# wbhart/mpir-fft

Measured on AMD Instinct MI355X. Metric: limbs/s for new_mpn_mul N×N-bit at 1/2/4/8 MI355X; % HBM roofline, higher is better.
Workload: dtype u64; 1 GPU; C3: new_mpn_mul depth=15 w=4 n1=n2=20312500 limbs (l=2048 limbs/coeff, NC x NR = 256 x 256, trunc=39936); parallelism=single

## Files before the change

include/mpfft.h:

```cpp
#ifndef MPFFT_H
#define MPFFT_H

#include <stddef.h>
#include <stdint.h>

#if !defined(__GMP_H__) && !defined(__MPIR_H__) && !defined(MPFFT_HAVE_MP_TYPES)
typedef uint64_t mp_limb_t;
typedef long mp_size_t;
typedef unsigned long mp_bitcnt_t;
#endif

#define MPFFT_VERSION 2

#define MPFFT_OK 0
#define MPFFT_EINVAL 1
#define MPFFT_ETOOBIG 2
#define MPFFT_EUNSUPPORTED 3
#define MPFFT_ENOMEM 4
#define MPFFT_EHIP 5
#define MPFFT_ENODEV 6

#ifdef __cplusplus
extern "C" {
#endif
// ... 83 lines not shown
    int src, dst;
    int op;
    int field;
    int src_layout, dst_layout;
    long src_off, dst_off, count;
} mpfft_copy;
#define MPFFT_XCHG_COL_TO_ROW 1
#define MPFFT_XCHG_ROW_TO_COL 2
#define MPFFT_LAYOUT_HALO 2
long mpfft_shard_exchange_plan(long n1, long n2, unsigned long depth, unsigned long w, int world, int which,
                               mpfft_copy *out, long cap);
long mpfft_shard_halo_plan(long n1, long n2, unsigned long depth, unsigned long w, int world,
                           mpfft_copy *out, long cap);

int mpfft_mul_multi(uint64_t *r1, const uint64_t *i1, long n1, const uint64_t *i2, long n2,
                    unsigned long depth, unsigned long w, int ngpus, const int *devices);

long mpfft_shard_src_limbs(long n1, long n2, unsigned long depth, unsigned long w, int world);
int mpfft_shard_pack(long n1, long n2, unsigned long depth, unsigned long w, int world, int rank,
                     const uint64_t *a, long na, uint64_t *out);

int mpfft_mul_multi_device(long n1, long n2, unsigned long depth, unsigned long w, int ngpus, const int *devices,
                           const uint64_t *const *d_src1, const uint64_t *const *d_src2, uint64_t *const *d_r,
                           void *const *streams);
int mpfft_multi_release(void);
long mpfft_multi_schedule(long n1, long n2, unsigned long depth, unsigned long w, int world, int calls, char *buf,
                          size_t len);

int mpfft_set_devices(int ngpus, const int *devices, long min_l);
int mpfft_last_ngpus(void);

int mpfft_profile_begin(int max_calls);
int mpfft_stage_kernels(long n1, long n2, unsigned long depth, unsigned long w, char *buf, size_t len);
int mpfft_profile_end(float *stage_ms, int *calls);

const char *mpfft_strerror(int code);
int mpfft_version(void);

void mpfft_fill_random(uint64_t *buf, long cnt, uint64_t seed);

#ifdef __cplusplus
}
#endif

#endif
```

mpir-fft_amd/__init__.py:

```python
import ctypes
import os

import numpy as np

_HERE = os.path.dirname(os.path.abspath(__file__))
_LIBSEL = os.environ.get("MPFFT_LIB", "")
LIB_PATH = os.path.join(_HERE, "libmpfft_diag.so" if _LIBSEL == "diag" else
                        _LIBSEL if _LIBSEL.endswith(".so") else "libmpfft.so")
_lib = None

STAGE_FWD_COLUMNS, STAGE_FWD_ROWS, STAGE_POINTWISE, STAGE_INV_ROWS, STAGE_INV_COLUMNS, \
    STAGE_SCALE, STAGE_COMBINE, STAGE_FOLD_COMBINE = range(8)

_u64p = ctypes.POINTER(ctypes.c_uint64)
_vp = ctypes.c_void_p
_L = ctypes.c_long
_UL = ctypes.c_ulong


class _Shard(ctypes.Structure):
    _fields_ = [("n1", ctypes.c_long), ("n2", ctypes.c_long), ("depth", ctypes.c_ulong), ("w", ctypes.c_ulong),
                ("c0", ctypes.c_int), ("ccount", ctypes.c_int), ("r0", ctypes.c_int), ("rcount", ctypes.c_int),
                ("ccb", ctypes.c_int),
                ("col_dig", ctypes.c_void_p * 2), ("col_cb", ctypes.c_void_p * 2), ("col_top", ctypes.c_void_p * 2),
# ... 250 lines not shown
def alloc_workspace(n1, n2, depth, w, device="cuda"):
    import torch
    nb = workspace_bytes(n1, n2, depth, w)
    if nb == 0:
        raise MpfftError(check_params(n1, n2, depth, w), "workspace")
    return torch.empty(nb, dtype=torch.uint8, device=device)


def mul_device(d_r, d_i1, n1, d_i2, n2, depth, w, ws, stream=None):
    rc = lib().mpfft_mul_device(_ptr(d_r), _ptr(d_i1), n1, _ptr(d_i2), n2, depth, w, _ptr(ws),
                                ws.numel() * ws.element_size(), _stream(stream))
    if rc:
        raise MpfftError(rc, "mpfft_mul_device")


def stage(which, d_i1, d_i2, d_r, n1, n2, depth, w, ws, stream=None):
    rc = lib().mpfft_stage(which, _ptr(d_i1), _ptr(d_i2), _ptr(d_r), n1, n2, depth, w, _ptr(ws),
                           ws.numel() * ws.element_size(), _stream(stream))
    if rc:
        raise MpfftError(rc, f"mpfft_stage({which})")


STAGE_NAMES = ("fwd_columns", "fwd_rows", "pointwise", "inv_rows", "inv_columns", "scale", "combine")


def stage_kernels(n1, n2, depth, w):
    buf = ctypes.create_string_buffer(512)
    rc = lib().mpfft_stage_kernels(n1, n2, depth, w, buf, len(buf))
    if rc:
        raise MpfftError(rc, "mpfft_stage_kernels")
    return dict(zip(STAGE_NAMES, buf.value.decode().split(";")))


def profile_begin(max_calls):
    rc = lib().mpfft_profile_begin(max_calls)
    if rc:
        raise MpfftError(rc, "mpfft_profile_begin")


def profile_end():
    ms = (ctypes.c_float * len(STAGE_NAMES))()
    calls = ctypes.c_int(0)
    rc = lib().mpfft_profile_end(ms, ctypes.byref(calls))
    if rc:
        raise MpfftError(rc, "mpfft_profile_end")
    return dict(zip(STAGE_NAMES, [float(x) for x in ms])), calls.value


def workspace_layout(n1, n2, depth, w):
    out = (ctypes.c_size_t * 8)()
    rc = lib().mpfft_workspace_layout(n1, n2, depth, w, out)
    if rc:
        raise MpfftError(rc, "workspace_layout")
    keys = ("digA", "topA", "cbA", "digB", "topB", "cbB", "slots", "cbw")
    return dict(zip(keys, list(out)))


def workspace_views(ws, n1, n2, depth, w):
    import torch
    P = plan_info(n1, n2, depth, w)
    lay = workspace_layout(n1, n2, depth, w)
    slots, l = lay["slots"], P["l"]
    u8 = ws.view(torch.uint8)

    def dig(off):
        return u8[off:off + slots * l * 8].view(torch.int64).view(slots, l)
# ... 158 lines not shown
```

mpir-fft_amd/csrc/kernels.hpp:

```cpp
#pragma once
#include "coeff.hpp"

struct PassArgs {
    u64 *dig[2];
    u64 *cb[2];
    int *top[2];
    const u64 *src[2];
    long nsrc[2];
    long src_chunk;
    u64 bits1;
    u64 N;
    int l;
    int lbM, lvl0;
    u64 rho;
    long sub_stride, pos_stride;
    int nsub, pos_off;
    int pbb;
    long pbs;
    int sub_off;
    long jNC;
    int zero_from;
    int need;
    int need_lo;
    int tw_mode;
    u64 tw_w;
    int tw_lbR;
    int canon;
    int ngroups;
    int nbuf;
    u64 scale_e;
    int ablate;
    unsigned *zp;
    long zn;
    unsigned long long *dbg;
    int pcarry;
    int pkeep;
    int fill_lo, fill_off;
    u64 fill_rho;
    int grp0;
};

__device__ inline void pass_clear_flags(const PassArgs &a)
{
    if (!a.zp) return;
    const long nt = (long)blockDim.x * blockDim.y * blockDim.z;
    const long nthr = (long)gridDim.x * gridDim.y * gridDim.z * nt;
    const long bid = ((long)blockIdx.z * gridDim.y + blockIdx.y) * gridDim.x + blockIdx.x;
    const long t = bid * nt + ((long)threadIdx.z * blockDim.y + threadIdx.y) * blockDim.x + threadIdx.x;
    for (long i = t; i < a.zn; i += nthr) a.zp[i] = 0u;
}

struct Lds {
    i64 *stage;
    int *edge;
    u64 *scr;
};

__host__ __device__ inline size_t lds_bytes(int l, int rb, int G, int U, int nw)
{
    size_t st = (size_t)rb * 2 * l * sizeof(i64);
    size_t ed = ((size_t)norm_edge_ints(G, U, nw) * sizeof(int) + 15) / 16 * 16;
    return st + ed + (size_t)norm_scr_u64(G, U, nw) * sizeof(u64);
}

template <int U, int G>
__device__ __forceinline__ Lds lds_carve(unsigned char *smem, int l, int rb, int nw)
{
    Lds d;
    d.stage = (i64 *)smem;
    unsigned char *p = smem + (size_t)rb * 2 * l * sizeof(i64);
    d.edge = (int *)p;
// ... 999 lines not shown
```

mpir-fft_amd/csrc/mpfft.hip:

```cpp
#include <hip/hip_runtime.h>
#include <stdint.h>
#include <stdio.h>
#include <stdlib.h>
#include <string.h>
#include <mutex>
#include <vector>

#include "kernels.hpp"
#include "combine.hpp"
#include "fold.hpp"
#include "wdispatch.hpp"
#include "bdispatch.hpp"
#include "pdispatch.hpp"
#include "rdispatch.hpp"
#include "../../include/mpfft.h"

static const char *diag_env(const char *name)
{
#ifdef MPFFT_DIAG
    return getenv(name);
#else
    (void)name;
    return nullptr;
#endif
}

static WvFns wv_fns(int U, bool full)
{
    switch (U) {
    case 1: return full ? wv_fns_u1_1() : wv_fns_u1_0();
    case 2: return full ? wv_fns_u2_1() : wv_fns_u2_0();
    case 3: return full ? wv_fns_u3_1() : wv_fns_u3_0();
    default: return full ? wv_fns_u4_1() : wv_fns_u4_0();
    }
}

struct Plan {
    long n1, n2;
// ... 262 lines not shown
static thread_local hipError_t last_hip_error = hipSuccess;
void mpfft_note_hip_error(hipError_t e) { last_hip_error = e; }

int mpfft_multi_policy(long n1, long n2, unsigned long depth, unsigned long w, std::vector<int> &devs);

struct View {
    u64 *dig[2];
    u64 *cb[2];
    int *top[2];
};

struct Exec {
    const Plan &P;
    hipStream_t s;
    int nw;
    View col, row;
    View cview = {};
    int c0, ccount, r0, rcount, ccb, cbb;
    long cbs;
    long src_chunk = 0;
    u32 *zflags = nullptr;
    long zflags_n = 0;
    int in_rows = 0;
    bool defer_double = false;
    bool fold = false;
    bool fuse_row_last = false;
    int own_lo = 0, own_hi = 0;
    bool carry_pend = !diag_env("MPFFT_NO_CARRY");
    int carry_mask() const
    {
        static const int m = [] { const char *e = diag_env("MPFFT_CARRY_MASK"); return e ? atoi(e) : -1; }();
        return m >= 0 ? m : 5;
    }
    struct Fill { long lo = 0, off = 0; u64 rho = 0; bool done = false; } fill;
    long dbl_lo = 0, dbl_hi = 0;

    Exec(const Plan &p, hipStream_t st) : P(p), s(st) { nw = P.tpb / 64; }

    int split(int rem, bool col = false, bool inv = false) const
    {
        const int ml = inv && P.maxlogg_i ? P.maxlogg_i : col && P.maxlogg_c ? P.maxlogg_c : P.maxlogg;
        const int np = (rem + ml - 1) / ml;
        return (rem + np - 1) / np;
    }

    static int comb_v()
    {
        static const int v = [] { const char *e = diag_env("MPFFT_CB_V"); const int x = e ? atoi(e) : 8;
                                  return x == 1 || x == 2 || x == 4 || x == 16 ? x : 8; }();
        return v;
    }
    static int comb_kw(const Plan &P) { return (int)((P.N + 32767) / P.bits1 + 1); }
    static bool comb_ct(const Plan &P)
    {
        static const bool no_ct = [] { const char *e = diag_env("MPFFT_COMB_CT"); return e && !strcmp(e, "0"); }();
        return comb_v() == 8 && !no_ct && comb_kw(P) <= 4;
    }
    static int comb_nt(const Plan &P)
    {
        static const int nt = [] { const char *e = diag_env("MPFFT_COMB_NT"); return e && atoi(e) == 256 ? 256 : 512; }();
        return comb_ct(P) ? nt : 256;
    }
    static long comb_blocks(const Plan &P, long mcount)
    {
        const long bl = (long)comb_nt(P) * comb_v();
        return (mcount + bl - 1) / bl;
    }
    u32 *comb_flags(unsigned char *ws) const { return (u32 *)(ws + P.off_flags); }
    static long comb_flag_words(const Plan &P, long mcount) { return (comb_blocks(P, mcount) + 4) / 4 * 4; }

    void single(unsigned char *ws)
    {
        col.dig[0] = (u64 *)(ws + P.off_digA);
        col.top[0] = (int *)(ws + P.off_topA);
        col.cb[0] = (u64 *)(ws + P.off_cbA);
        col.dig[1] = (u64 *)(ws + P.off_digB);
        col.top[1] = (int *)(ws + P.off_topB);
        col.cb[1] = (u64 *)(ws + P.off_cbB);
        row = col;
        if (P.has_c) {
            cview.dig[0] = (u64 *)(ws + P.off_digC);
            cview.top[0] = (int *)(ws + P.off_topC);
            cview.cb[0] = (u64 *)(ws + P.off_cbC);
        }
        c0 = 0;
        ccount = (int)P.NC;
        r0 = 0;
        rcount = (int)P.Tr;
        ccb = (int)P.NC;
        cbb = P.lbC;
        cbs = (long)P.Tr * P.NC;
    }

    void shift(long slots)
    {
        const long cbw = cb_words((int)P.l);
        for (int k = 0; k < 2; ++k) {
            col.dig[k] += slots * P.l;
            col.cb[k] += slots * cbw;
            col.top[k] += slots;
        }
        row = col;
        if (cview.dig[0]) {
            cview.dig[0] += slots * P.l;
            cview.cb[0] += slots * cbw;
            cview.top[0] += slots;
        }
    }

    int stage_bufs(int G) const
    {
        long fit = (64L * 1024) / (16L * P.l);
        if (fit < 1) fit = 1;
        return (int)(fit < G ? fit : G);
    }

    int rpass_mode(const PassArgs &a, int logg, int dir) const
    {
        if (!P.rpass || logg > (dir ? rp_maxlogg_dit((int)P.l) : rp_maxlogg_fwd4((int)P.l)) || a.canon || a.rho % 128) return -1;
        if (dir == 0) {
            if (a.scale_e || a.tw_mode == 2) return -1;
            if (a.src[0] || a.src[1]) return a.tw_mode || a.pcarry ? -1 : 2;
            if (a.zero_from < (1 << a.lbM)) return -1;
            if (a.tw_mode == 1) return a.pcarry ? -1 : 1;
// ... 10 lines not shown
    int rp_mode(const PassArgs &a, int logg, int dir) const
    {
        int rm = rpass_mode(a, logg, dir);
        static const int rmask = [] { const char *e = diag_env("MPFFT_RPASS_OFF"); return e ? atoi(e) : 0; }();
        if (rm >= 0 && (rmask >> (4 * dir + rm) & 1)) rm = -1;
        return rm;
    }

    template <typename MK>
    int fit(int k, int dir, MK mk) const
    {
        if (!P.big || !P.bp_lg || k <= P.bp_lg || rp_mode(mk(k), k, dir) >= 0) return k;
        return P.bp_lg;
    }

    static void live_groups(PassArgs &a, int logg, int dir)
    {
        a.ngroups = 1 << (a.lbM - logg);
        a.grp0 = 0;
        if (dir != 0) return;
        const int slg = a.lbM - a.lvl0, lobits = slg - logg;
        const long nh = 1L << a.lvl0;
        const long hlo = std::min<long>(nh, a.need_lo > 0 ? (long)a.need_lo >> slg : 0);
        const long hhi = std::min<long>(nh, ((long)a.need + (1L << slg) - 1) >> slg);
        if (hhi > hlo) {
            a.grp0 = (int)(hlo << lobits);
            a.ngroups = (int)((hhi - hlo) << lobits);
        }
    }

    int pass(PassArgs a, int logg, int dir, int nops)
    {
        const int rm = rp_mode(a, logg, dir);
        if (rm >= 0) {
            rp_fn f = rp_get((int)P.l, logg, dir, rm);
            if (!f) return MPFFT_EUNSUPPORTED;
            static const size_t pad = [] { const char *e = diag_env("MPFFT_RPASS_LDSPAD"); return e ? (size_t)atol(e) : 0; }();
            static const int abl = [] { const char *e = diag_env("MPFFT_ABLATE"); return e ? atoi(e) : 0; }();
            a.ablate = abl;
            const size_t lds = rp_lds((int)P.l, logg) + pad;
            allow_lds((const void *)f, lds);
            live_groups(a, logg, dir);
            dim3 grid((unsigned)((long)a.nsub * a.ngroups), (unsigned)nops);
            static const bool stamps = diag_env("MPFFT_RP_STAMPS") != nullptr;
            const unsigned nt = (unsigned)rp_nt((int)P.l, logg, dir);
            if (stamps) return bp_stamped(f, grid, nt, lds, a, logg, dir);
            hipLaunchKernelGGL(f, grid, dim3(nt), lds, s, a);
            HIPCHK(hipGetLastError());
            return MPFFT_OK;
        }
        if (P.big) {
            const bool gen = (a.rho % 64) || (a.tw_mode && a.tw_w % 64) || (a.scale_e % 64);
            bp_fn f = gen ? bp_get_gen(logg, dir) : bp_get(logg, dir);
            if (!f) return MPFFT_EUNSUPPORTED;
            const size_t lds = bp_lds_need((int)P.l, 1 << logg);
            allow_lds((const void *)f, lds);
            live_groups(a, logg, dir);
            dim3 grid((unsigned)((long)a.nsub * a.ngroups), (unsigned)nops);
            const unsigned nthr = (unsigned)(64 * bp_waves((int)P.l, logg));
            static const bool stamps = diag_env("MPFFT_BP_STAMPS") != nullptr;
            if (stamps) return bp_stamped(f, grid, nthr, lds, a, logg, dir);
            hipLaunchKernelGGL(f, grid, dim3(nthr), lds, s, a);
            HIPCHK(hipGetLastError());
            return MPFFT_OK;
        }
        if (P.wave && P.lds) {
// ... 352 lines not shown
    int ifft_block(long off, long m)
    {
        if (int rc = flush_chain()) return rc;
        const int lbM = ilog2(m);
        int hi = lbM;
        while (hi > 0) {
            auto mk = [&](int kk) {
                PassArgs b = col_args();
                b.lbM = lbM;
                b.lvl0 = hi - kk;
                b.rho = rho_blk(m);
                b.pos_off = (int)off;
                b.zero_from = (int)m;
                b.need = (int)m;
                if (P.fuse_scale && hi - kk == 0 && m == P.NR) {
                    b.scale_e = 2 * P.N - (u64)(P.depth + 1);
                    b.canon = 1;
                }
                if (fold && P.ltw && hi == lbM) {
                    b.tw_mode = 3;
                    b.tw_w = (u64)P.w;
                    b.tw_lbR = P.lbR;
                    b.scale_e = 2 * P.N - (u64)(P.depth + 1);
                }
                return b;
            };
            const int k = fit(split(hi, true, true), 1, mk);
            PassArgs a = mk(k);
            if (hi - k == 0 && fill.off) {
                PassArgs f = a;
                f.fill_lo = (int)fill.lo;
                f.fill_off = (int)fill.off;
                f.fill_rho = fill.rho;
                if (rp_mode(f, k, 1) >= 0) {
                    a = f;
                    fill.done = true;
                }
            }
            int rc = pass(a, k, 1, 1);
            if (rc) return rc;
            hi -= k;
        }
        return MPFFT_OK;
    }

    struct Chain { long off = 0, t = 0; int n = 0; long h[3] = {0, 0, 0}; } chain;

    int flush_chain()
    {
        const Chain c = chain;
        chain.n = 0;
        for (int j = 0; j < c.n; ++j) {
            int rc = pairop_now(OP_TWOXMY, c.off, c.h[j], 0, c.t, 0);
            if (rc) return rc;
        }
        return MPFFT_OK;
    }

    PairArgs pair_args(int op, long off, long h, long i0, long cnt, u64 rho) const
    {
        PairArgs a;
        memset(&a, 0, sizeof(a));
        a.dig = col.dig[0];
        a.cb = col.cb[0];
        a.top = col.top[0];
        a.N = P.N;
        a.l = (int)P.l;
        a.op = op;
        a.NC = ccount;
        a.ncol = ccount;
        a.off = (int)off;
        a.h = (int)h;
        a.i0 = (int)i0;
        a.cnt = (int)cnt;
        a.rho = rho;
        return a;
    }

    int pairop(int op, long off, long h, long i0, long cnt, u64 rho)
    {
        if (cnt <= 0) return MPFFT_OK;
        int rc;
        const bool chains = P.rpass && rp_chain_get((int)P.l, 1) && !diag_env("MPFFT_NO_CHAIN");
        if (chains && op == OP_TWOXMY && i0 == 0) {
            if (chain.n && (chain.off != off || chain.t != cnt || chain.n == 3) && (rc = flush_chain())) return rc;
            if (!chain.n) {
                chain.off = off;
                chain.t = cnt;
            }
            chain.h[chain.n++] = h;
            return MPFFT_OK;
        }
        if (chains && op == OP_IBFLY && i0 == 0 && chain.n && chain.off == off + h && chain.t == cnt) {
            PairArgs a = pair_args(op, off + h, h, 0, cnt, rho);
            a.nb = chain.n;
            for (int j = 0; j < chain.n; ++j) a.hb[j] = (int)chain.h[j];
            a.xoff = (int)off;
            rp_pair_fn f = rp_chain_get((int)P.l, chain.n);
            chain.n = 0;
            hipLaunchKernelGGL(f, dim3((unsigned)(cnt * ccount)), dim3(RP_NT), rp_chain_lds((int)P.l), s, a);
            HIPCHK(hipGetLastError());
            return MPFFT_OK;
        }
        if ((rc = flush_chain())) return rc;
        return pairop_now(op, off, h, i0, cnt, rho);
    }

    int pairop_now(int op, long off, long h, long i0, long cnt, u64 rho)
    {
        if (cnt <= 0) return MPFFT_OK;
        PairArgs a;
        a.dig = col.dig[0];
        a.cb = col.cb[0];
        a.top = col.top[0];
        a.N = P.N;
        a.l = (int)P.l;
        a.op = op;
        a.NC = ccount;
        a.ncol = ccount;
        a.off = (int)off;
        a.h = (int)h;
        a.i0 = (int)i0;
        a.cnt = (int)cnt;
        a.rho = rho;
        if (P.rpass) {
            rp_pair_fn f = rp_pair_get((int)P.l, op);
            if (!f) return MPFFT_EUNSUPPORTED;
            hipLaunchKernelGGL(f, dim3((unsigned)(cnt * ccount)), dim3(RP_NT), rp_pair_lds((int)P.l), s, a);
            HIPCHK(hipGetLastError());
            return MPFFT_OK;
        }
        if (P.wave) {
            void (*f)(PairArgs) = wv_fns(P.wU, P.wfull).pair;
            const size_t lds = (size_t)WPB * 16 * P.l;
            allow_lds((const void *)f, lds);
            const long waves = cnt * ccount;
            hipLaunchKernelGGL(f, dim3((unsigned)((waves + WPB - 1) / WPB)), dim3(64 * WPB), lds, s, a);
            HIPCHK(hipGetLastError());
            return MPFFT_OK;
        }
        const size_t lds = lds_bytes((int)P.l, 2, 2, P.U, nw);
        void (*f)(PairArgs) = nullptr;
        switch (P.U) {
// ... 5 lines not shown
        hipLaunchKernelGGL(f, dim3((unsigned)(cnt * ccount)), dim3(P.tpb), lds, s, a);
        HIPCHK(hipGetLastError());
        return MPFFT_OK;
    }

    u64 rho_blk(long m) const { return (u64)P.w * P.NC * (u64)(P.NR / m); }

    int itft(long off, long m, long t)
    {
        int rc = itft_r(off, m, t);
        return rc ? rc : flush_chain();
    }
    int itft1(long off, long m, long t)
    {
        int rc = itft1_r(off, m, t);
        return rc ? rc : flush_chain();
    }

    int itft_r(long off, long m, long t)
    {
        int rc;
        const long h = m / 2;
        const bool top = defer_double && off == 0 && m == P.NR;
        if (t == m) return ifft_block(off, m);
        if (t <= h) {
            if ((rc = itft_r(off, h, t))) return rc;
            if (top) {
                dbl_lo = 0;
                dbl_hi = t;
                return MPFFT_OK;
            }
            return pairop(OP_DOUBLE, off, h, 0, t, 0);
        }
        fill = {t - h, h, rho_blk(m), false};
        rc = ifft_block(off, h);
        const bool filled = fill.done;
        fill = {};
        if (rc) return rc;
        if (!filled && (rc = pairop(OP_FILL, off, h, t - h, h - (t - h), rho_blk(m)))) return rc;
        if ((rc = itft1_r(off + h, h, t - h))) return rc;
        if ((rc = pairop(OP_IBFLY, off, h, 0, t - h, rho_blk(m)))) return rc;
        if (top) {
            dbl_lo = t - h;
            dbl_hi = h;
            return MPFFT_OK;
        }
        return pairop(OP_DOUBLE, off, h, t - h, h - (t - h), 0);
    }

    int itft1_r(long off, long m, long t)
    {
        int rc;
        const long h = m / 2;
        if (t == m) return ifft_block(off, m);
        if (t <= h) {
            if ((rc = pairop(OP_HALFADD, off, h, t, h - t, 0))) return rc;
            if ((rc = itft1_r(off, h, t))) return rc;
            return pairop(OP_TWOXMY, off, h, 0, t, 0);
        }
        if ((rc = ifft_block(off, h))) return rc;
        if ((rc = pairop(OP_FIX, off, h, t - h, h - (t - h), rho_blk(m)))) return rc;
        if ((rc = itft1_r(off + h, h, t - h))) return rc;
        return pairop(OP_IBFLY, off, h, 0, t - h, rho_blk(m));
    }

    int scale()
    {
        if (P.fuse_scale || fold) return MPFFT_OK;
        const u64 e = 2 * P.N - (u64)(P.depth + 1);
        if (dbl_hi <= dbl_lo) return scale_rows(0, P.Tr, e);
        if (P.rpass) return scale_rows(0, P.Tr, e, dbl_lo, dbl_hi);
        int rc;
        if ((rc = scale_rows(0, dbl_lo, e))) return rc;
        if ((rc = scale_rows(dbl_lo, dbl_hi, e + 1))) return rc;
        return scale_rows(dbl_hi, P.Tr, e);
    }

    int scale_rows(long r0_, long r1_, u64 e, long d0 = 0, long d1 = 0)
    {
        const long cnt = (r1_ - r0_) * ccount, s0 = r0_ * ccount;
        if (cnt <= 0) return MPFFT_OK;
        u64 *dig = col.dig[0] + s0 * P.l, *cbp = col.cb[0] + s0 * cb_words((int)P.l);
        int *top = col.top[0] + s0;
        if (P.rpass) {
            static const int snt_env = [] { const char *e = diag_env("MPFFT_SCALE_NT"); return e ? atoi(e) : 0; }();
            const int snt = snt_env == 256 || snt_env == 512 ? snt_env : P.l <= 2048 ? 256 : 512;
            rp_scale_fn f = rp_scale_get((int)P.l, snt);
            if (!f) return MPFFT_EUNSUPPORTED;
            const unsigned lo = (unsigned)((d0 - r0_) * ccount), hi = (unsigned)((d1 - r0_) * ccount);
            hipLaunchKernelGGL(f, dim3((unsigned)cnt), dim3(snt), rp_scale_lds((int)P.l), s, dig, cbp, top, (unsigned)P.N,
// ... 216 lines not shown
        XC.col = XC.row = X1.col;
    }
    if ((rc = X1.inv_rows())) return rc;
    if (two && (rc = X2.inv_rows())) return rc;
    pc.mark(4, s);
    if ((rc = X1.itft(0, P.NR, P.NR))) return rc;
    if (two) {
        if ((rc = s2_launch(P, X1, S2_FILL, nullptr, nullptr, P2.Tr * P.NC, (P.NR - P2.Tr) * P.NC, 0, 1))) return rc;
        if ((rc = X2.itft1(0, P.NR, P2.Tr))) return rc;
    }
    if ((rc = s2_launch(P, X1, S2_IBFLY, nullptr, nullptr, 0, 2 * P.n, tlo > 0 ? tlo : 0, 1))) return rc;
    pc.mark(5, s);
    if ((rc = XS.scale())) return rc;
    pc.mark(6, s);
    rc = XC.combine_single(d_r, ws);
    pc.mark(7, s);
    return rc;
}

struct HostB {
    const u64 *h;
    hipStream_t cs;
    hipEvent_t ready;
};

static int run_all(const Plan &P, u64 *d_r, const u64 *d_i1, const u64 *d_i2, unsigned char *ws, hipStream_t s,
                   const HostB *hb = nullptr)
{
    if (P.sqrt2) return run_all6(P, d_r, d_i1, d_i2, ws, s);
    Exec X(P, s);
    X.single(ws);
    X.zflags = X.comb_flags(ws);
    X.zflags_n = X.comb_flag_words(P, P.total);
    X.defer_double = true;
    X.fold = P.fold != 0;
    X.fuse_row_last = true;
    ProfCall pc;
    int rc;
    pc.mark(0, s);
    if (hb && hb->h) {
        if ((rc = X.fwd_columns(d_i1, P.n1, d_i2, P.n2, 1, 0))) return rc;
        if ((rc = X.fwd_rows(1, 0))) return rc;
        HIPCHK(hipMemcpyAsync((void *)d_i2, hb->h, (size_t)P.n2 * 8, hipMemcpyHostToDevice, hb->cs));
        HIPCHK(hipEventRecord(hb->ready, hb->cs));
        HIPCHK(hipStreamWaitEvent(s, hb->ready, 0));
        if ((rc = X.fwd_columns(d_i1, P.n1, d_i2, P.n2, 1, 1))) return rc;
        if ((rc = X.fwd_rows(1, 1))) return rc;
        pc.mark(1, s);
    } else {
        if ((rc = X.fwd_columns(d_i1, P.n1, d_i2, P.n2, 2))) return rc;
        pc.mark(1, s);
        if ((rc = X.fwd_rows(2))) return rc;
    }
    pc.mark(2, s);
    if ((rc = X.pointwise())) return rc;
    pc.mark(3, s);
    if ((rc = X.inv_rows())) return rc;
    pc.mark(4, s);
    if ((rc = X.itft(0, P.NR, P.Tr))) return rc;
    pc.mark(5, s);
    if ((rc = X.scale())) return rc;
    pc.mark(6, s);
    rc = X.fold ? X.combine_fold(d_r, ws, X.dbl_lo, X.dbl_hi) : X.combine_single(d_r, ws);
    pc.mark(7, s);
    return rc;
}

extern "C" {

int mpfft_stage_kernels(long n1, long n2, unsigned long depth, unsigned long w, char *buf, size_t len)
{
    Plan P;
    int rc = make_plan(&P, n1, n2, depth, w);
    if (rc) return rc;
    const char *pass = P.big ? (P.rpass ? "k_rpass" : "k_bpass") : (P.wave && P.lds) ? "k_lpass" : P.wave ? "k_wpass" : "k_pass";
    char pw[96];
    const int lk = Exec::pwss_lk(P.l);
    const char *rows = P.big && P.rpass && !(lk && pw_get(pw_inner_limbs(P.l, lk), lk)) ? "k_rpass + k_bpass (canonical last pass)" : pass;
    const char *fz = diag_env("MPFFT_FUSE_ROW");
    const bool fused = P.has_c && !(fz && !strcmp(fz, "0"));
    if (lk && pw_get(pw_inner_limbs(P.l, lk), lk))
        snprintf(pw, sizeof pw, "k_pwss<%d>%s (nested negacyclic, K=%d)", pw_inner_limbs(P.l, lk),
                 !fused ? "" : P.fuse_rows == 2 ? " quad + last two row levels" : " pair + last row level", 1 << lk);
    else if (P.l % 256 == 0 && P.l <= 4096 && pw_kind() != PW_MFMA1 && pw_kind() != PW_VALU)
        snprintf(pw, sizeof pw, "k_pwm2 (int8 MFMA)");
    else if (P.l % 128 == 0 && pw_kind() != PW_VALU)
        snprintf(pw, sizeof pw, "k_pwm (int8 MFMA)");
    else if (P.l % 2 == 0 && P.l >= 32)
        snprintf(pw, sizeof pw, "k_pw (VALU)");
    else
        snprintf(pw, sizeof pw, "k_pointwise (VALU)");
    const char *pair = P.rpass ? "k_rpair" : P.wave ? "k_wpair" : "k_pairop";
    const char *scale = P.fuse_scale ? "(fused into the last inverse column pass)"
                        : P.fold ? "(folded: 2^-(depth+1) in the last inverse row pass)"
                        : P.rpass ? "k_rscale" : P.wave ? "k_wscale" : "k_scale";
    const char *comb = P.fold ? "k_cmeta + k_combine_red (reduced form)" : "k_combine1";
    snprintf(buf, len, "%s;%s;%s;%s;%s + %s;%s;%s", pass, rows, pw, pass, pass, pair, scale, comb);
    return MPFFT_OK;
}

int mpfft_profile_begin(int max_calls)
{
    std::lock_guard<std::mutex> lk(g_prof_mu);
    if (max_calls < 1 || g_prof.inflight > 0) return MPFFT_EINVAL;
    const int per = MPFFT_NSTAGES + 1;
    if (g_prof.cap < max_calls) {
        for (int i = 0; i < g_prof.cap * per; ++i) (void)hipEventDestroy(g_prof.ev[i]);
        free(g_prof.ev);
        free(g_prof.marks);
        g_prof.cap = 0;
        g_prof.ev = (hipEvent_t *)calloc((size_t)max_calls * per, sizeof(hipEvent_t));
        g_prof.marks = (int *)calloc((size_t)max_calls, sizeof(int));
        if (!g_prof.ev || !g_prof.marks) return MPFFT_ENOMEM;
        for (int i = 0; i < max_calls * per; ++i)
            if (hipEventCreate(&g_prof.ev[i]) != hipSuccess) {
                for (int j = 0; j < i; ++j) (void)hipEventDestroy(g_prof.ev[j]);
                return MPFFT_EHIP;
            }
        g_prof.cap = max_calls;
    }
    for (int c = 0; c < g_prof.cap; ++c) g_prof.marks[c] = 0;
    g_prof.used = 0;
    g_prof.on = true;
    return MPFFT_OK;
}

int mpfft_profile_end(float *stage_ms, int *calls)
{
    std::lock_guard<std::mutex> lk(g_prof_mu);
    g_prof.on = false;
// ... 60 lines not shown
    int rc = make_plan(&P, n1, n2, depth, w);
    if (rc) return rc;
    out[0] = P.n; out[1] = P.l; out[2] = P.NC; out[3] = P.j1; out[4] = P.j2;
    out[5] = P.trunc; out[6] = (long)P.bits1; out[7] = P.NR; out[8] = P.tpb; out[9] = P.U;
    return MPFFT_OK;
}

int mpfft_mul_device(uint64_t *d_r, const uint64_t *d_i1, long n1, const uint64_t *d_i2, long n2,
                     unsigned long depth, unsigned long w, void *d_ws, size_t ws_bytes, void *stream)
{
    Plan P;
    int rc = make_plan(&P, n1, n2, depth, w);
    if (rc) return rc;
    if (!d_ws || ws_bytes < P.bytes) return MPFFT_ENOMEM;
    (void)hipGetLastError();
    return run_all(P, d_r, d_i1, d_i2, (unsigned char *)d_ws, (hipStream_t)stream);
}

int mpfft_stage(int stage, const uint64_t *d_i1, const uint64_t *d_i2, uint64_t *d_r, long n1, long n2,
                unsigned long depth, unsigned long w, void *d_ws, size_t ws_bytes, void *stream)
{
    Plan P;
    int rc = make_plan(&P, n1, n2, depth, w);
    if (rc) return rc;
    if (!d_ws || ws_bytes < P.bytes) return MPFFT_ENOMEM;
    (void)hipGetLastError();
    Exec X(P, (hipStream_t)stream);
    X.single((unsigned char *)d_ws);
    switch (stage) {
    case MPFFT_STAGE_FWD_COLUMNS: return X.fwd_columns(d_i1, n1, d_i2, n2, 2);
    case MPFFT_STAGE_FWD_ROWS: return X.fwd_rows(2);
    case MPFFT_STAGE_POINTWISE: return X.pointwise();
    case MPFFT_STAGE_INV_ROWS: return X.inv_rows();
    case MPFFT_STAGE_INV_COLUMNS: return X.itft(0, P.NR, P.Tr);
    case MPFFT_STAGE_SCALE: return X.scale();
    case MPFFT_STAGE_COMBINE: return X.combine_single(d_r, (unsigned char *)d_ws);
    case MPFFT_STAGE_FOLD_COMBINE: {
        if (!P.fold) return MPFFT_EUNSUPPORTED;
        long lo, hi;
        plan_dbl(P, &lo, &hi);
        return X.combine_fold(d_r, (unsigned char *)d_ws, lo, hi);
    }
    }
    return MPFFT_EINVAL;
}

static int shard_exec(Exec &X, const mpfft_shard *sh)
{
    const Plan &P = X.P;
    if (sh->ccount < 1 || sh->c0 < 0 || sh->c0 + sh->ccount > P.NC) return MPFFT_EINVAL;
    if (sh->rcount < 0 || sh->r0 < 0 || sh->r0 + sh->rcount > P.Tr) return MPFFT_EINVAL;
    if (sh->ccb < 1 || P.NC % sh->ccb || (sh->ccb & (sh->ccb - 1))) return MPFFT_EINVAL;
    for (int k = 0; k < 2; ++k) {
        X.col.dig[k] = sh->col_dig[k];
        X.col.cb[k] = sh->col_cb[k];
        X.col.top[k] = sh->col_top[k];
        X.row.dig[k] = sh->row_dig[k];
        X.row.cb[k] = sh->row_cb[k];
        X.row.top[k] = sh->row_top[k];
    }
    X.c0 = sh->c0;
    X.ccount = sh->ccount;
    X.r0 = sh->r0;
    X.rcount = sh->rcount;
    X.ccb = sh->ccb;
    X.cbb = ilog2(sh->ccb);
    X.cbs = (long)sh->rcount * sh->ccb;
// ... 353 lines not shown
```

mpir-fft_amd/csrc/rkernels.hpp:

```cpp
#pragma once
#include "bkernels.hpp"
#include "rdispatch.hpp"

typedef unsigned long long rp_v2u __attribute__((ext_vector_type(2)));

#define RP_FENCE() do { asm volatile("" ::: "memory"); __builtin_amdgcn_sched_barrier(0); } while (0)

__device__ __forceinline__ u32 rp_uniform(u32 v) { return (u32)__builtin_amdgcn_readfirstlane((int)v); }

__device__ __forceinline__ int rp_launder(int t)
{
    asm volatile("" : "+v"(t));
    return t;
}

typedef unsigned int rp_v4u __attribute__((ext_vector_type(4)));

struct Pr {
    u32 w[4];
    int h;
};

__device__ __forceinline__ Pr pr_make(rp_v4u v, int h)
{
// ... 240 lines not shown
}

__device__ __forceinline__ u32 rp_mod2n(u32 e, u32 N2)
{
    e = e >= 2 * N2 ? e - 2 * N2 : e;
    return e >= N2 ? e - N2 : e;
}

template <int LOGG, int DIR>
__device__ __forceinline__ u32 rp_tw(const PassArgs &a, const BGeo &g, int li, int k)
{
    const int JB = DIR == 0 ? LOGG - 1 - li : li;
    const int level = DIR == 0 ? a.lvl0 + li : a.lvl0 + LOGG - 1 - li;
    const u32 h = 1u << (a.lbM - level - 1);
    const u32 unit = (u32)a.rho << level;
    return (u32)(g.pos0 & (h - 1)) * unit + (u32)(k & ((1 << JB) - 1)) * (u32)g.pstep * unit;
}

__device__ __forceinline__ u32 rp_pend_pos(u32 rho, int lbM, int lo, int hi, u32 p, u32 N2)
{
    const u32 xm = p & ((1u << (lbM - hi)) - 1);
    u32 e = 0;
    for (int lev = lo; lev < hi; ++lev)
        if ((p >> (lbM - lev - 1)) & 1) e = rp_mod2n(e + (rho << lev) * xm, N2);
    return e;
}

template <int LOGG>
__device__ __forceinline__ u32 rp_pend(const PassArgs &a, const BGeo &g, int done, int s, u32 N2)
{
    return rp_pend_pos((u32)a.rho, a.lbM, a.lvl0 - a.pcarry, a.lvl0 + done, (u32)(g.pos0 + s * g.pstep), N2);
}

template <int G, int PP, int NX, int NT = RP_NT, typename EF>
__device__ __forceinline__ void rp_rot_all(Pr (&x)[G][rp_r(PP, NT)], const RX<PP> &X, EF efn, u32 N, int t)
{
    t = rp_launder(t);
#pragma unroll
    for (int i0 = 0; i0 < G; i0 += NX) {
#pragma unroll
        for (int q = 0; q < NX && i0 + q < G; ++q) rp_pub<PP, NT>(X, q, x[i0 + q], t);
        __syncthreads();
#pragma unroll
        for (int q = 0; q < NX && i0 + q < G; ++q) {
            const u32 e = efn(i0 + q);
            if (e == 0) continue;
#pragma unroll
            for (int r = 0; r < rp_r(PP, NT); ++r) {
                RP_FENCE();
                x[i0 + q][r] = rp_get_rot<PP>(X, q, t + NT * r, e, N);
            }
        }
        __syncthreads();
    }
}

template <int LOGG, int DIR, bool GX, bool CIN = false>
__device__ __forceinline__ u32 rp_exp_entry(const PassArgs &a0, const BGeo &g, int e, u32 N2, u32 cadd)
{
    constexpr int G = 1 << LOGG;
    PassArgs a = a0;
    if (CIN) a.pcarry = 0;
    if (e < G) {
        if (CIN) return rp_pend_pos((u32)a0.rho, a0.lbM, a0.lvl0 - a0.pcarry, a0.lvl0, (u32)(g.pos0 + e * g.pstep), N2);
        if (DIR == 1 && a.tw_mode == 3) {
            const long row = (long)a.pos_off + g.pos0 + (long)e * g.pstep;
            const u64 t = bp_mod2n(g.tw0 * (u64)revbin_dev(row, a.tw_lbR), N2);
            return (u32)bp_mod2n((t ? N2 - t : 0) + a.scale_e, N2);
        }
        if (!GX) return 0;
        return DIR == 0 ? (u32)bp_mod2n(g.tw0 + (u64)e * g.twst + cadd, N2) : (u32)bp_post(a, g, e, N2);
    }
    if (e < 2 * G) return DIR == 0 ? rp_pend<LOGG>(a, g, LOGG, e - G, N2) : 0;
    e -= 2 * G;
// ... 421 lines not shown
            const int k = i | (1 << JB);
            if (pz(k)) {
#pragma unroll
                for (int r = 0; r < R; ++r) x[k][r] = x[i][r];
                continue;
            }
            const u32 E = rp_uniform(EXPT[2 * G + (G / 2) * li + pi]);
#pragma unroll
            for (int r = 0; r < R; ++r) {
                if (r % 2 == 0) RP_FENCE();
                bool ng;
                const Pr y = rp_get_al<PP>(X, pi, tl + NT * r, E, N, ng);
                pr_bfly(x[i][r], x[k][r], x[i][r], y, ng);
            }
        }
        if (xch) __syncthreads();
        if (li < 3) RP_STAMP(2 + li);
    }
    if (DIR == 0 && !a.pkeep && a.lvl0 + LOGG < a.lbM) {
        rp_rot_all_al<G, PP, NX, NT>(x, X, [&](int s) -> u32 { return rp_uniform(EXPT[G + s]); }, N, t);
    }
    if (DIR == 1) rp_pin<G, R>(x);
    if (DIR == 1 && GX) {
        rp_rot_all<G, PP, NX, NT>(x, X, [&](int s) -> u32 { return rp_uniform(EXPT[s]); }, N, t);
    }
    RP_STAMP(5);

    if (DIR == 1) rp_pin<G, R>(x);
    rp_store<G, G, PP, NT>(x, st, SLT, [&](int i) -> bool {
        const int bs = (g.pos0 + i * g.pstep) & ~(g.pstep - 1);
        return DIR == 1 || (bs < a.need && bs + g.pstep > a.need_lo);
    }, (short *)smem, t);
    if (FILL) {
        auto fills = [&](int s) -> bool { return g.pos0 + s * g.pstep >= a.fill_lo; };
        __syncthreads();
        if (t < G) SLT[t] += (u32)((long)a.fill_off * a.pos_stride);
        rp_rot_all_al<G, PP, NX, NT>(x, X, [&](int s) -> u32 {
            return fills(s) ? (u32)(((u64)(g.pos0 + s * g.pstep) * a.fill_rho) % N2) : 0u;
        }, N, t);
        rp_store<G, G, PP, NT>(x, st, SLT, fills, (short *)smem, t);
    }
    RP_STAMP(6);
    if (stamp) {
        __syncthreads();
        RP_STAMP(7);
    }
#undef RP_STAMP
}

template <int PP, int OP>
__global__ __launch_bounds__(RP_NT) void k_rpair(PairArgs a)
{
    constexpr int l = 1024 * PP;
    constexpr bool LOADB = OP != OP_DOUBLE && OP != OP_FILL;
    extern __shared__ __attribute__((aligned(16))) unsigned char smem[];
    const RX<PP> X{smem};
    u32 *SL = (u32 *)(smem + RX<PP>::SB);
    const int t = threadIdx.x;
    const int col = (int)(blockIdx.x % a.ncol);
    const int i = a.i0 + (int)(blockIdx.x / a.ncol);
    const u32 N = (u32)a.N, N2 = 2 * (u32)a.N;
    const u32 e = (u32)(((u64)i * a.rho) % N2);
    if (t < 2) SL[t] = (u32)((long)(a.off + i + (t ? a.h : 0)) * a.NC + col);
    __syncthreads();
    Coef st;
    st.dig = a.dig;
    st.cb = a.cb;
    st.top = a.top;
    unsigned short *CODE = (unsigned short *)smem;
    Pr x[2][PP];
    const RpCodes cd = rp_codes_load<LOADB ? 2 : 1, PP>(st, SL, t);
    rp_load_limbs<LOADB ? 2 : 1, 2, PP>(x, st, SL, t);
    rp_codes_store<LOADB ? 2 : 1, PP>(CODE, cd, t);
// ... 272 lines not shown
```

Before: 5.385 billion limbs/s.

## Fold tail half-add steps into the FILL inverse-column pass

During the truncated inverse column transform, the FILL epilogue of the last radix pass now also performs the OP_HALFADD accumulation for small strides, adjusting the fill rotation exponents to compensate. The matching separate half-add pair launches are then skipped. This removes extra full passes over the coefficient buffer, at the cost of more complex in-kernel bookkeeping and extra adds in the FILL path. A schedule-recording mode and API were also added to list the inverse-column launches.

```diff
diff --git a/include/mpfft.h b/include/mpfft.h
--- a/include/mpfft.h
+++ b/include/mpfft.h
@@ -139,6 +139,7 @@
 
 int mpfft_profile_begin(int max_calls);
 int mpfft_stage_kernels(long n1, long n2, unsigned long depth, unsigned long w, char *buf, size_t len);
+int mpfft_inv_columns_schedule(long n1, long n2, unsigned long depth, unsigned long w, char *buf, size_t len);
 int mpfft_profile_end(float *stage_ms, int *calls);
 
 const char *mpfft_strerror(int code);
diff --git a/mpir-fft_amd/__init__.py b/mpir-fft_amd/__init__.py
--- a/mpir-fft_amd/__init__.py
+++ b/mpir-fft_amd/__init__.py
@@ -306,6 +306,17 @@
     return dict(zip(STAGE_NAMES, buf.value.decode().split(";")))
 
 
+def inv_columns_schedule(n1, n2, depth, w):
+    f = lib().mpfft_inv_columns_schedule
+    f.argtypes = [_L, _L, _UL, _UL, ctypes.c_char_p, ctypes.c_size_t]
+    f.restype = ctypes.c_int
+    buf = ctypes.create_string_buffer(1 << 16)
+    rc = f(n1, n2, depth, w, buf, len(buf))
+    if rc:
+        raise MpfftError(rc, "mpfft_inv_columns_schedule")
+    return buf.value.decode().splitlines()
+
+
 def profile_begin(max_calls):
     rc = lib().mpfft_profile_begin(max_calls)
     if rc:
diff --git a/mpir-fft_amd/csrc/kernels.hpp b/mpir-fft_amd/csrc/kernels.hpp
--- a/mpir-fft_amd/csrc/kernels.hpp
+++ b/mpir-fft_amd/csrc/kernels.hpp
@@ -37,6 +37,7 @@
     int pkeep;
     int fill_lo, fill_off;
     u64 fill_rho;
+    int fill_hmin;
     int grp0;
 };
 
diff --git a/mpir-fft_amd/csrc/mpfft.hip b/mpir-fft_amd/csrc/mpfft.hip
--- a/mpir-fft_amd/csrc/mpfft.hip
+++ b/mpir-fft_amd/csrc/mpfft.hip
@@ -4,6 +4,7 @@
 #include <stdlib.h>
 #include <string.h>
 #include <mutex>
+#include <string>
 #include <vector>
 
 #include "kernels.hpp"
@@ -332,7 +333,9 @@
         static const int m = [] { const char *e = diag_env("MPFFT_CARRY_MASK"); return e ? atoi(e) : -1; }();
         return m >= 0 ? m : 5;
     }
-    struct Fill { long lo = 0, off = 0; u64 rho = 0; bool done = false; } fill;
+    struct Fill { long lo = 0, off = 0; u64 rho = 0; bool done = false; long hmin = 0, habs = 0; } fill;
+    bool tail_fold = false;
+    std::string *rec = nullptr;
     long dbl_lo = 0, dbl_hi = 0;
 
     Exec(const Plan &p, hipStream_t st) : P(p), s(st) { nw = P.tpb / 64; }
@@ -369,8 +372,26 @@
     u32 *comb_flags(unsigned char *ws) const { return (u32 *)(ws + P.off_flags); }
     static long comb_flag_words(const Plan &P, long mcount) { return (comb_blocks(P, mcount) + 4) / 4 * 4; }
 
+    void drive_single()
+    {
+        defer_double = true;
+        tail_fold = true;
+        fold = P.fold != 0;
+    }
+
     void single(unsigned char *ws)
     {
+        c0 = 0;
+        ccount = (int)P.NC;
+        r0 = 0;
+        rcount = (int)P.Tr;
+        ccb = (int)P.NC;
+        cbb = P.lbC;
+        cbs = (long)P.Tr * P.NC;
+        if (!ws) {
+            col = row = cview = View{};
+            return;
+        }
         col.dig[0] = (u64 *)(ws + P.off_digA);
         col.top[0] = (int *)(ws + P.off_topA);
         col.cb[0] = (u64 *)(ws + P.off_cbA);
@@ -383,13 +404,6 @@
             cview.top[0] = (int *)(ws + P.off_topC);
             cview.cb[0] = (u64 *)(ws + P.off_cbC);
         }
-        c0 = 0;
-        ccount = (int)P.NC;
-        r0 = 0;
-        rcount = (int)P.Tr;
-        ccb = (int)P.NC;
-        cbb = P.lbC;
-        cbs = (long)P.Tr * P.NC;
     }
 
     void shift(long slots)
@@ -466,6 +480,17 @@
     int pass(PassArgs a, int logg, int dir, int nops)
     {
         const int rm = rp_mode(a, logg, dir);
+        if (rec) {
+            char ln[160];
+            int n = rm >= 0 ? snprintf(ln, sizeof ln, "k_rpass<%d,%d,%d,%d> pos %d+%d", logg, (int)P.l / 1024, dir, rm, a.pos_off, 1 << a.lbM)
+                            : snprintf(ln, sizeof ln, "pass<%d,%d> pos %d+%d", logg, dir, a.pos_off, 1 << a.lbM);
+            if (rm >= 0 && !rp_get((int)P.l, logg, dir, rm)) return MPFFT_EUNSUPPORTED;
+            if (a.fill_off) n += snprintf(ln + n, sizeof ln - n, " fill lo=%d off=%d", a.fill_lo, a.fill_off);
+            if (a.fill_hmin) n += snprintf(ln + n, sizeof ln - n, " halfadd %d..%d", a.fill_off / 2, a.fill_hmin);
+            *rec += ln;
+            *rec += '\n';
+            return MPFFT_OK;
+        }
         if (rm >= 0) {
             rp_fn f = rp_get((int)P.l, logg, dir, rm);
             if (!f) return MPFFT_EUNSUPPORTED;
@@ -884,9 +909,13 @@
                 f.fill_lo = (int)fill.lo;
                 f.fill_off = (int)fill.off;
                 f.fill_rho = fill.rho;
-                if (rp_mode(f, k, 1) >= 0) {
+                const long hm = std::max(fill.hmin, 1L << (lbM - k));
+                if (fill.hmin && hm <= fill.off / 2) f.fill_hmin = (int)hm;
+                const int fm = rp_mode(f, k, 1);
+                if (fm >= 0 && rp_get((int)P.l, k, 1, fm)) {
                     a = f;
                     fill.done = true;
+                    fill.habs = f.fill_hmin;
                 }
             }
             int rc = pass(a, k, 1, 1);
@@ -950,6 +979,12 @@
             a.xoff = (int)off;
             rp_pair_fn f = rp_chain_get((int)P.l, chain.n);
             chain.n = 0;
+            if (rec) {
+                char ln[96];
+                snprintf(ln, sizeof ln, "k_rchain<%d,%d> off=%ld h=%ld cnt=%ld\n", (int)P.l / 1024, a.nb, off + h, h, cnt);
+                *rec += ln;
+                return MPFFT_OK;
+            }
             hipLaunchKernelGGL(f, dim3((unsigned)(cnt * ccount)), dim3(RP_NT), rp_chain_lds((int)P.l), s, a);
             HIPCHK(hipGetLastError());
             return MPFFT_OK;
@@ -961,6 +996,13 @@
     int pairop_now(int op, long off, long h, long i0, long cnt, u64 rho)
     {
         if (cnt <= 0) return MPFFT_OK;
+        if (rec) {
+            char ln[96];
+            if (P.rpass) snprintf(ln, sizeof ln, "k_rpair<%d,%d> off=%ld h=%ld i0=%ld cnt=%ld\n", (int)P.l / 1024, op, off, h, i0, cnt);
+            else snprintf(ln, sizeof ln, "pair<%d> off=%ld h=%ld i0=%ld cnt=%ld\n", op, off, h, i0, cnt);
+            *rec += ln;
+            return MPFFT_OK;
+        }
         PairArgs a;
         a.dig = col.dig[0];
         a.cb = col.cb[0];
@@ -1032,13 +1074,17 @@
             }
             return pairop(OP_DOUBLE, off, h, 0, t, 0);
         }
-        fill = {t - h, h, rho_blk(m), false};
+        long hmin = 0;
+        if (tail_fold)
+            for (long d = h / 2; d > t - h; d /= 2) hmin = d;
+        fill = {t - h, h, rho_blk(m), false, hmin, 0};
         rc = ifft_block(off, h);
         const bool filled = fill.done;
+        const long habs = fill.habs;
         fill = {};
         if (rc) return rc;
         if (!filled && (rc = pairop(OP_FILL, off, h, t - h, h - (t - h), rho_blk(m)))) return rc;
-        if ((rc = itft1_r(off + h, h, t - h))) return rc;
+        if ((rc = itft1_r(off + h, h, t - h, habs))) return rc;
         if ((rc = pairop(OP_IBFLY, off, h, 0, t - h, rho_blk(m)))) return rc;
         if (top) {
             dbl_lo = t - h;
@@ -1048,14 +1094,14 @@
         return pairop(OP_DOUBLE, off, h, t - h, h - (t - h), 0);
     }
 
-    int itft1_r(long off, long m, long t)
+    int itft1_r(long off, long m, long t, long habs = 0)
     {
         int rc;
         const long h = m / 2;
         if (t == m) return ifft_block(off, m);
         if (t <= h) {
-            if ((rc = pairop(OP_HALFADD, off, h, t, h - t, 0))) return rc;
-            if ((rc = itft1_r(off, h, t))) return rc;
+            if (!(habs && h >= habs) && (rc = pairop(OP_HALFADD, off, h, t, h - t, 0))) return rc;
+            if ((rc = itft1_r(off, h, t, habs))) return rc;
             return pairop(OP_TWOXMY, off, h, 0, t, 0);
         }
         if ((rc = ifft_block(off, h))) return rc;
@@ -1338,8 +1384,7 @@
     X.single(ws);
     X.zflags = X.comb_flags(ws);
     X.zflags_n = X.comb_flag_words(P, P.total);
-    X.defer_double = true;
-    X.fold = P.fold != 0;
+    X.drive_single();
     X.fuse_row_last = true;
     ProfCall pc;
     int rc;
@@ -1372,7 +1417,30 @@
     return rc;
 }
 
+static std::string inv_columns_launches(const Plan &P)
+{
+    std::string out;
+    if (P.sqrt2) return out;
+    Exec X(P, nullptr);
+    X.single(nullptr);
+    X.drive_single();
+    X.rec = &out;
+    if (X.itft(0, P.NR, P.Tr)) out.clear();
+    return out;
+}
+
 extern "C" {
+
+int mpfft_inv_columns_schedule(long n1, long n2, unsigned long depth, unsigned long w, char *buf, size_t len)
+{
+    Plan P;
+    int rc = make_plan(&P, n1, n2, depth, w);
+    if (rc) return rc;
+    const std::string s = inv_columns_launches(P);
+    if (!buf || s.size() + 1 > len) return MPFFT_EINVAL;
+    memcpy(buf, s.c_str(), s.size() + 1);
+    return MPFFT_OK;
+}
 
 int mpfft_stage_kernels(long n1, long n2, unsigned long depth, unsigned long w, char *buf, size_t len)
 {
@@ -1401,7 +1469,15 @@
                         : P.fold ? "(folded: 2^-(depth+1) in the last inverse row pass)"
                         : P.rpass ? "k_rscale" : P.wave ? "k_wscale" : "k_scale";
     const char *comb = P.fold ? "k_cmeta + k_combine_red (reduced form)" : "k_combine1";
-    snprintf(buf, len, "%s;%s;%s;%s;%s + %s;%s;%s", pass, rows, pw, pass, pass, pair, scale, comb);
+    char invc[96];
+    int d1 = 0, d0 = 0;
+    const std::string sched = inv_columns_launches(P);
+    const size_t ha = sched.find(" halfadd ");
+    if (ha != std::string::npos && sscanf(sched.c_str() + ha, " halfadd %d..%d", &d1, &d0) == 2)
+        snprintf(invc, sizeof invc, "%s (FILL + half-add d=%d..%d) + %s", pass, d1, d0, pair);
+    else
+        snprintf(invc, sizeof invc, "%s + %s", pass, pair);
+    snprintf(buf, len, "%s;%s;%s;%s;%s;%s;%s", pass, rows, pw, pass, invc, scale, comb);
     return MPFFT_OK;
 }
 
@@ -1528,7 +1604,7 @@
     case MPFFT_STAGE_FWD_ROWS: return X.fwd_rows(2);
     case MPFFT_STAGE_POINTWISE: return X.pointwise();
     case MPFFT_STAGE_INV_ROWS: return X.inv_rows();
-    case MPFFT_STAGE_INV_COLUMNS: return X.itft(0, P.NR, P.Tr);
+    case MPFFT_STAGE_INV_COLUMNS: X.tail_fold = true; return X.itft(0, P.NR, P.Tr);
     case MPFFT_STAGE_SCALE: return X.scale();
     case MPFFT_STAGE_COMBINE: return X.combine_single(d_r, (unsigned char *)d_ws);
     case MPFFT_STAGE_FOLD_COMBINE: {
diff --git a/mpir-fft_amd/csrc/rkernels.hpp b/mpir-fft_amd/csrc/rkernels.hpp
--- a/mpir-fft_amd/csrc/rkernels.hpp
+++ b/mpir-fft_amd/csrc/rkernels.hpp
@@ -296,14 +296,15 @@
     return rp_pend_pos((u32)a.rho, a.lbM, a.lvl0 - a.pcarry, a.lvl0 + done, (u32)(g.pos0 + s * g.pstep), N2);
 }
 
-template <int G, int PP, int NX, int NT = RP_NT, typename EF>
+template <int G, int PP, int NX, int NT = RP_NT, bool SK = false, typename EF>
 __device__ __forceinline__ void rp_rot_all(Pr (&x)[G][rp_r(PP, NT)], const RX<PP> &X, EF efn, u32 N, int t)
 {
     t = rp_launder(t);
 #pragma unroll
     for (int i0 = 0; i0 < G; i0 += NX) {
 #pragma unroll
-        for (int q = 0; q < NX && i0 + q < G; ++q) rp_pub<PP, NT>(X, q, x[i0 + q], t);
+        for (int q = 0; q < NX && i0 + q < G; ++q)
+            if (!SK || efn(i0 + q)) rp_pub<PP, NT>(X, q, x[i0 + q], t);
         __syncthreads();
 #pragma unroll
         for (int q = 0; q < NX && i0 + q < G; ++q) {
@@ -791,13 +792,46 @@
         return DIR == 1 || (bs < a.need && bs + g.pstep > a.need_lo);
     }, (short *)smem, t);
     if (FILL) {
-        auto fills = [&](int s) -> bool { return g.pos0 + s * g.pstep >= a.fill_lo; };
+        if (t < G) {
+            const int p = g.pos0 + t * g.pstep;
+            u32 e = 0, keep = 0;
+            if (p >= a.fill_lo) {
+                int q = p, c = 0;
+                for (int d = a.fill_off >> 1; a.fill_hmin && d >= a.fill_hmin; d >>= 1) {
+                    if (q >= a.fill_lo + d && q < 2 * d) {
+                        q -= d;
+                        ++c;
+                    } else if (q < d) {
+                        ++c;
+                    }
+                }
+                e = rp_mod2n((u32)(((u64)p * a.fill_rho) % N2) + N2 - (u32)c, N2);
+                keep = q == p;
+            }
+            EXPT[t] = e;
+            EXPT[G + t] = keep;
+        }
         __syncthreads();
         if (t < G) SLT[t] += (u32)((long)a.fill_off * a.pos_stride);
-        rp_rot_all_al<G, PP, NX, NT>(x, X, [&](int s) -> u32 {
-            return fills(s) ? (u32)(((u64)(g.pos0 + s * g.pstep) * a.fill_rho) % N2) : 0u;
-        }, N, t);
-        rp_store<G, G, PP, NT>(x, st, SLT, fills, (short *)smem, t);
+        constexpr bool FPIN = PP == 4 && LOGG == 3;
+        if (FPIN) rp_pin<G, R>(x);
+        rp_rot_all<G, PP, NX, NT, true>(x, X, [&](int s) -> u32 { return rp_uniform(EXPT[s]); }, N, t);
+        if (FPIN) rp_pin<G, R>(x);
+        if (a.fill_hmin) {
+#pragma unroll
+            for (int dl = LOGG - 1; dl >= 0; --dl) {
+                const int ds = 1 << dl;
+                if (ds * g.pstep < a.fill_hmin) continue;
+#pragma unroll
+                for (int s = 0; s < ds; ++s) {
+                    if (g.pos0 + s * g.pstep < a.fill_lo) continue;
+#pragma unroll
+                    for (int r = 0; r < R; ++r) x[s][r] = pr_add(x[s][r], x[s + ds][r]);
+                }
+            }
+            if (FPIN) rp_pin<G, R>(x);
+        }
+        rp_store<G, G, PP, NT>(x, st, SLT, [&](int s) -> bool { return rp_uniform(EXPT[G + s]) != 0; }, (short *)smem, t);
     }
     RP_STAMP(6);
     if (stamp) {
```

Result: faster. 5.471 billion limbs/s (median of 6 runs) (+1.6%).
